# stateless-consensus/phant

Hardware: NVIDIA H100
Metric: mpt_proofs_verified_per_sec (higher is better)
Workload: dtype u64

## Files before the change

### phant_b200/csrc/abi.cu

```cuda
#include "../../include/phant_gpu.h"
#include "common.cuh"
#include "ctx.cuh"

#include <cub/device/device_scan.cuh>

#include <stdio.h>
#include <stdlib.h>
#include <string.h>
#include <new>

using namespace phant;

#define CU(expr)                                                              \
    do {                                                                      \
        cudaError_t e_ = (expr);                                              \
        if (e_ != cudaSuccess) return ctx->fail(e_, #expr, __FILE__, __LINE__); \
    } while (0)

int phant_gpu_ctx::fail(cudaError_t e, const char* what, const char* file, int line)
{
    snprintf(last_error, sizeof last_error, "%s: %s (%s:%d)", cudaGetErrorName(e), what, file, line);
    cudaGetLastError();
    return e == cudaErrorMemoryAllocation ? PHANT_GPU_E_OOM : PHANT_GPU_E_CUDA;
}
// ... 190 lines not shown
    stats.launches++;
    stats.keccak_msgs += n;
    stats.keccak_bytes += total_bytes;
    return PHANT_GPU_OK;
}

int phant_gpu_ctx::hash_slots(const uint8_t* d_msgs, const uint64_t* d_off, const uint64_t* d_len, uint64_t n, uint8_t* d_out)
{
    phant_gpu_ctx* ctx = this;
    if (n == 0) return PHANT_GPU_OK;
    KeccakVariant variant = KECCAK_STAGED;
    if (flags & PHANT_GPU_FLAG_KECCAK_DIRECT) variant = KECCAK_DIRECT;
    if (flags & PHANT_GPU_FLAG_KECCAK_WARP) variant = KECCAK_WARP;
    if (variant == KECCAK_STAGED && ((uintptr_t)d_msgs & 15)) variant = KECCAK_DIRECT;
    time_begin(0);
    CU(launch_keccak(stream, device, variant, d_msgs, d_off, nullptr, n, d_out, nullptr, d_len));
    time_end();
    stats.launches++;
    stats.keccak_msgs += n;
    return PHANT_GPU_OK;
}

bool phant_gpu_ctx::fused_ok(const uint8_t* d_nodes, uint64_t n_proofs, uint64_t n_nodes) const
{
    const uint32_t other = PHANT_GPU_FLAG_UNFUSED_WALK | PHANT_GPU_FLAG_KECCAK_DIRECT | PHANT_GPU_FLAG_KECCAK_WARP;
    return !(flags & other) && !((uintptr_t)d_nodes & 15) && !walk_peer && n_proofs <= 0xffffffffull && n_nodes <= 0xffffffffull;
}

int phant_gpu_ctx::verify_fused(const uint8_t* d_nodes, const uint64_t* d_node_off, uint64_t n_nodes, uint64_t total_bytes,
                                const uint64_t* d_proof_first, uint64_t np, const uint8_t* d_keys, const uint8_t* d_roots, uint64_t n_roots,
                                uint64_t* d_bitmap, uint8_t* d_status, uint64_t* d_voff, uint32_t* d_vlen)
{
    phant_gpu_ctx* ctx = this;
    if (np == 0) return wait_walk_fence();
    NvtxRange nvtx("phant:hash+walk");
    if (int rc = d_perms.reserve(ctx, 64)) return rc;
    if (!perms_init) { CU(cudaMemsetAsync(d_perms.ptr, 0, 64, stream)); perms_init = true; }
    const uint32_t* order = nullptr;
    if (!(flags & PHANT_GPU_FLAG_NO_BINNING) && np >= 4096) {
        if (int rc = d_idx.reserve(ctx, keccak_regroup_scratch_bytes(device, np))) return rc;
        if (int rc = d_order.reserve(ctx, 4 * np)) return rc;
        CU(launch_keccak_classify(stream, device, d_proof_first, np, (uint32_t*)d_idx.ptr, (uint32_t*)((unsigned long long*)d_perms.ptr + 1),
                                  nullptr, true));
        CU(launch_keccak_regroup(stream, device, d_proof_first, np, (const uint32_t*)d_idx.ptr, (uint32_t*)d_order.ptr, true));
        stats.launches += 2;
        order = (const uint32_t*)d_order.ptr;
    }
    if (!d_status) {
        if (int rc = ctx->d_status.reserve(ctx, np)) return rc;
        d_status = (uint8_t*)ctx->d_status.ptr;
    }
    time_begin(0);
    CU(launch_verify_fused(stream, device, d_nodes, d_node_off, d_proof_first, order, np, d_keys, d_roots, n_roots, d_status, d_voff, d_vlen,
                           (unsigned long long*)d_perms.ptr));
    time_end();
    stats.launches++;
    stats.keccak_msgs += n_nodes;
    stats.keccak_bytes += total_bytes;
    perms_pending = true;
    if (int rc = wait_walk_fence()) return rc;
    if (d_bitmap) {
        time_begin(1);
        CU(launch_verdict(stream, device, d_status, np, d_bitmap));
        time_end();
        stats.launches++;
    }
    return PHANT_GPU_OK;
}

static int check_offsets_host(const uint64_t* off, uint64_t n, uint64_t* total)
{
    for (uint64_t i = 0; i < n; ++i)
        if (off[i + 1] < off[i]) return PHANT_GPU_E_INVALID;
    *total = off[n];
    return PHANT_GPU_OK;
}

extern "C" int phant_gpu_keccak256_batch(phant_gpu_ctx* ctx, const uint8_t* msgs, const uint64_t* off, uint64_t n, uint8_t* out)
{
    if (!ctx || (n && (!off || !out))) return PHANT_GPU_E_INVALID;
    if (n == 0) return PHANT_GPU_OK;
    CU(cudaSetDevice(ctx->device));
    if (ctx->flags & PHANT_GPU_FLAG_DEVICE_PTRS) {
        uint64_t last = 0;
        CU(cudaMemcpyAsync(&last, off + n, 8, cudaMemcpyDeviceToHost, ctx->stream));
        CU(cudaStreamSynchronize(ctx->stream));
        if (last && !msgs) return PHANT_GPU_E_INVALID;
        return ctx->hash_csr(msgs, off, n, last, out);
    }
    uint64_t total = 0;
    if (int rc = check_offsets_host(off, n, &total)) return rc;
    if (total && !msgs) return PHANT_GPU_E_INVALID;
    if (int rc = ctx->d_msgs.reserve(ctx, total + 64)) return rc;
    if (int rc = ctx->d_off.reserve(ctx, 8 * (n + 1))) return rc;
    if (int rc = ctx->d_out.reserve(ctx, 32 * n)) return rc;
    if (total) CU(cudaMemcpyAsync(ctx->d_msgs.ptr, msgs, total, cudaMemcpyHostToDevice, ctx->stream));
    CU(cudaMemcpyAsync(ctx->d_off.ptr, off, 8 * (n + 1), cudaMemcpyHostToDevice, ctx->stream));
    ctx->stats.h2d_bytes += total + 8 * (n + 1);
    if (int rc = ctx->hash_csr((const uint8_t*)ctx->d_msgs.ptr, (const uint64_t*)ctx->d_off.ptr, n, total, (uint8_t*)ctx->d_out.ptr)) return rc;
    CU(cudaMemcpyAsync(out, ctx->d_out.ptr, 32 * n, cudaMemcpyDeviceToHost, ctx->stream));
    ctx->stats.d2h_bytes += 32 * n;
    CU(cudaStreamSynchronize(ctx->stream));
    return PHANT_GPU_OK;
}

extern "C" int phant_gpu_keccak256_batch_async(phant_gpu_ctx* ctx, const uint8_t* msgs, const uint64_t* off, uint64_t n, uint64_t total_bytes,
                                               uint8_t* out)
// ... 501 lines not shown
```

### phant_b200/csrc/common.cuh

```cuda
#pragma once
#include <cuda_runtime.h>
#include <stdint.h>

namespace phant {

enum KeccakVariant { KECCAK_STAGED = 0, KECCAK_DIRECT = 1, KECCAK_WARP = 2 };

int keccak_num_sms(int device);
cudaError_t launch_keccak(cudaStream_t s, int device, KeccakVariant variant, const uint8_t* msgs, const uint64_t* off,
                          const uint32_t* order, uint64_t n, uint8_t* out, uint32_t* summary ,
                          const uint64_t* len = nullptr );
uint64_t keccak_regroup_scratch_bytes(int device, uint64_t n);
cudaError_t launch_keccak_classify(cudaStream_t s, int device, const uint64_t* off, uint64_t n, uint32_t* hist, uint32_t* ticket,
                                   unsigned long long* perms, bool proofs = false);
cudaError_t launch_keccak_regroup(cudaStream_t s, int device, const uint64_t* off, uint64_t n, const uint32_t* start, uint32_t* order,
                                  bool proofs = false);
cudaError_t launch_verify_fused(cudaStream_t s, int device, const uint8_t* nodes, const uint64_t* node_off, const uint64_t* proof_first,
                                const uint32_t* order, uint64_t n, const uint8_t* keys32, const uint8_t* roots32, uint64_t n_roots,
                                uint8_t* status, uint64_t* val_off , uint32_t* val_len , unsigned long long* perms);

constexpr int PEER_MAX_WORLD = 16;
struct PeerOut {
    uint32_t* dst[PEER_MAX_WORLD];
    unsigned long long* ready[PEER_MAX_WORLD];
    const unsigned long long* done;
    unsigned long long wait_done;
    unsigned long long step;
    uint32_t* ticket;
    uint32_t* err;
    uint32_t world;
};

cudaError_t launch_walk(cudaStream_t s, int device, uint64_t n_proofs, const uint8_t* nodes, const uint64_t* node_off,
                        const uint64_t* node_index , const uint64_t* proof_first, const uint8_t* keys32, const uint8_t* roots32, uint64_t n_roots,
                        const uint8_t* digests, const uint32_t* summary , uint64_t* bitmap, uint8_t* status,
                        uint64_t* val_off, uint32_t* val_len, const PeerOut* peer = nullptr );

cudaError_t launch_verdict(cudaStream_t s, int device, const uint8_t* status, uint64_t n, uint64_t* bitmap);

cudaError_t launch_peer_collect(cudaStream_t s, const unsigned long long* ready, uint32_t world, unsigned long long step, const void* src, void* dst,
                                uint64_t bytes, const PeerOut& sig);

cudaError_t launch_bag_build(cudaStream_t s, int device, const uint8_t* digests, uint64_t n_nodes, uint32_t* table, uint32_t capacity);
cudaError_t launch_walk_bag(cudaStream_t s, int device, uint64_t n_keys, const uint8_t* nodes, const uint64_t* node_off, const uint8_t* keys32,
                            const uint8_t* roots32, uint64_t n_roots, const uint8_t* digests, const uint32_t* summary, const uint32_t* table,
                            uint32_t capacity, uint64_t* bitmap, uint8_t* status, uint64_t* val_off, uint32_t* val_len);

struct StateOut {
    uint8_t* account_status;
    uint64_t* nonce;
    uint8_t* balance32;
    uint8_t* storage_root32;
    uint8_t* code_hash32;
    uint32_t* code_index;
    uint8_t* slot_status;
    uint8_t* slot_vals32;
};
cudaError_t launch_read_accounts(cudaStream_t s, int device, uint64_t n_accounts, const uint8_t* nodes, const uint64_t* node_off,
                                 const uint8_t* digests, const uint32_t* summary, const uint32_t* table, uint32_t capacity,
                                 const uint8_t* keys32, const uint8_t* roots32, uint64_t n_roots, const uint8_t* code_digests,
                                 const uint32_t* code_table , uint32_t code_capacity, uint8_t* rec_roots32,
                                 uint8_t* rec_status, const StateOut& out);
cudaError_t launch_read_slots(cudaStream_t s, int device, uint64_t n_slots, const uint8_t* nodes, const uint64_t* node_off,
                              const uint8_t* digests, const uint32_t* summary, const uint32_t* table, uint32_t capacity,
                              const uint8_t* keys32, const uint32_t* slot_account, uint64_t n_accounts, const uint8_t* rec_roots32,
                              const uint8_t* rec_status, const StateOut& out);

cudaError_t launch_synth_c2(cudaStream_t s, int device, uint64_t seed, uint64_t first_index, uint64_t n, uint32_t depth,
                            int corrupt, uint8_t* nodes, uint64_t* node_off, uint64_t* proof_first, uint8_t* keys32,
                            uint8_t* roots32);
cudaError_t launch_synth_c3_sizes(cudaStream_t s, int device, uint64_t seed, uint64_t first_index, uint64_t n,
                                  uint64_t* n_nodes_per, uint64_t* n_bytes_per);
// ... 7 lines not shown
```

### phant_b200/csrc/keccak_f1600.cuh

```cuda
#pragma once
#include <stdint.h>

namespace phant {

__constant__ uint64_t KECCAK_RC[24] = {
    0x0000000000000001ull, 0x0000000000008082ull, 0x800000000000808aull, 0x8000000080008000ull,
    0x000000000000808bull, 0x0000000080000001ull, 0x8000000080008081ull, 0x8000000000008009ull,
    0x000000000000008aull, 0x0000000000000088ull, 0x0000000080008009ull, 0x000000008000000aull,
    0x000000008000808bull, 0x800000000000008bull, 0x8000000000008089ull, 0x8000000000008003ull,
    0x8000000000008002ull, 0x8000000000000080ull, 0x000000000000800aull, 0x800000008000000aull,
    0x8000000080008081ull, 0x8000000000008080ull, 0x0000000080000001ull, 0x8000000080008008ull};

constexpr int KECCAK_RATE = 136;
constexpr int KECCAK_RATE_WORDS = 17;

template <int N>
__device__ __forceinline__ uint64_t rol64(uint64_t x)
{
    if constexpr (N == 0) return x;
    const uint32_t lo = (uint32_t)x, hi = (uint32_t)(x >> 32);
    uint32_t rlo, rhi;
    if constexpr (N == 32) {
        rlo = hi; rhi = lo;
    } else if constexpr (N < 32) {
// ... 65 lines not shown
__device__ __forceinline__ MsgView msg_view(const void* p)
{
    const uintptr_t a = (uintptr_t)p;
    return MsgView{(const uint64_t*)(a & ~(uintptr_t)7), (uint32_t)(a & 7) * 8};
}
__device__ __forceinline__ uint64_t funnel64(uint64_t lo, uint64_t hi, uint32_t sh)
{
    return sh ? (lo >> sh) | (hi << (64 - sh)) : lo;
}

template <int UNROLL>
__device__ __forceinline__ void absorb_full(uint64_t (&st)[25], const MsgView& v, uint32_t base)
{
    uint64_t w[KECCAK_RATE_WORDS + 1];
#pragma unroll
    for (int k = 0; k < KECCAK_RATE_WORDS; ++k) w[k] = v.w[base + k];
    w[KECCAK_RATE_WORDS] = v.sh ? v.w[base + KECCAK_RATE_WORDS] : 0;
#pragma unroll
    for (int k = 0; k < KECCAK_RATE_WORDS; ++k) st[k] ^= funnel64(w[k], w[k + 1], v.sh);
    keccak_f1600<UNROLL>(st);
}

template <int UNROLL>
__device__ __forceinline__ void absorb_final(uint64_t (&st)[25], const MsgView& v, uint32_t base, uint32_t rem)
{
    const uint32_t mis = v.sh >> 3;
#pragma unroll
    for (int k = 0; k < KECCAK_RATE_WORDS; ++k) {
        const int valid = (int)rem - 8 * k;
        uint64_t word = 0;
        if (valid > 0) {
            const uint64_t lo = v.w[base + k];
            const uint64_t hi = (mis + (valid > 8 ? 8 : valid) > 8) ? v.w[base + k + 1] : 0;
            word = funnel64(lo, hi, v.sh);
            if (valid < 8) word &= (1ull << (8 * valid)) - 1;
        }
        if (valid >= 0 && valid < 8) word ^= 1ull << (8 * valid);
        st[k] ^= word;
    }
    st[KECCAK_RATE_WORDS - 1] ^= 0x8000000000000000ull;
    keccak_f1600<UNROLL, true>(st);
}

#ifndef PHANT_HOST_SMEM
__device__ __forceinline__ uint32_t lds32(uint32_t saddr)
{
    uint32_t v;
    asm volatile("ld.shared.u32 %0, [%1];" : "=r"(v) : "r"(saddr));
    return v;
}
#else
__device__ __forceinline__ uint32_t lds32(uint32_t saddr) { uint32_t v; memcpy(&v, PHANT_HOST_SMEM + saddr, 4); return v; }
#endif
template <int UNROLL, bool DIGEST_ONLY = false>
__device__ __forceinline__ void absorb_full_smem(uint64_t (&st)[25], uint32_t sa)
{
    const uint32_t a4 = sa & ~3u, sh = (sa & 3u) * 8;
    uint32_t w[2 * KECCAK_RATE_WORDS + 1];
#pragma unroll
    for (int j = 0; j < 2 * KECCAK_RATE_WORDS; ++j) w[j] = lds32(a4 + 4 * j);
    w[2 * KECCAK_RATE_WORDS] = sh ? lds32(a4 + 4 * 2 * KECCAK_RATE_WORDS) : 0;
#pragma unroll
    for (int k = 0; k < KECCAK_RATE_WORDS; ++k) {
        const uint32_t lo = __funnelshift_r(w[2 * k], w[2 * k + 1], sh);
        const uint32_t hi = __funnelshift_r(w[2 * k + 1], w[2 * k + 2], sh);
        st[k] ^= ((uint64_t)hi << 32) | lo;
    }
    keccak_f1600<UNROLL, DIGEST_ONLY>(st);
}
#ifndef PHANT_HOST_SMEM
__device__ __forceinline__ void sts32_(uint32_t saddr, uint32_t v) { asm volatile("st.shared.u32 [%0], %1;" ::"r"(saddr), "r"(v) : "memory"); }
#else
__device__ __forceinline__ void sts32_(uint32_t saddr, uint32_t v) { memcpy(PHANT_HOST_SMEM + saddr, &v, 4); }
#endif
template <int UNROLL>
__device__ __forceinline__ void absorb_final_smem_masked(uint64_t (&st)[25], uint32_t sa, uint32_t rem)
{
    const uint32_t a4 = sa & ~3u, sh = (sa & 3u) * 8;
    const uint32_t nfw = rem >> 2, tail = rem & 3u;
    const uint32_t bmask = (1u << (8 * tail)) - 1u, pad = 1u << (8 * tail);
    uint32_t prev = rem ? lds32(a4) : 0;
#pragma unroll
    for (int j = 0; j < 2 * KECCAK_RATE_WORDS; ++j) {
        uint32_t word = 0;
        if ((uint32_t)j < nfw || ((uint32_t)j == nfw && tail)) {
            const uint32_t next = lds32(a4 + 4 * (j + 1));
            word = __funnelshift_r(prev, next, sh);
            prev = next;
        }
        if ((uint32_t)j == nfw) word = (word & bmask) ^ pad;
        if (j == 2 * KECCAK_RATE_WORDS - 1) word ^= 0x80000000u;
        st[j >> 1] ^= (j & 1) ? ((uint64_t)word << 32) : (uint64_t)word;
    }
    keccak_f1600<UNROLL, true>(st);
}
template <int UNROLL>
__device__ __forceinline__ void absorb_final_smem(uint64_t (&st)[25], uint32_t sa, uint32_t rem, uint32_t room)
{
    if (room < KECCAK_RATE + 4) { absorb_final_smem_masked<UNROLL>(st, sa, rem); return; }
    const uint32_t a4 = sa & ~3u, s = sa & 3u;
    const uint32_t p0 = rem + s, p1 = KECCAK_RATE - 1 + s;
    const uint32_t q0 = p0 >> 2, b0 = p0 & 3u, q1 = p1 >> 2, b1 = p1 & 3u;
    uint32_t w0 = lds32(a4 + 4 * q0);
    w0 = (w0 & ((1u << (8 * b0)) - 1u)) | (1u << (8 * b0));
    if (q0 == q1) w0 |= 0x80u << (8 * b1);
    sts32_(a4 + 4 * q0, w0);
    for (uint32_t q = q0 + 1; q < q1; ++q) sts32_(a4 + 4 * q, 0u);
    if (q1 > q0) sts32_(a4 + 4 * q1, 0x80u << (8 * b1));
    absorb_full_smem<UNROLL, true>(st, sa);
}

template <int UNROLL = 2>
__device__ __forceinline__ void keccak256_thread(const uint8_t* p, uint64_t len, uint64_t (&digest)[4])
{
    uint64_t st[25];
#pragma unroll
    for (int i = 0; i < 25; ++i) st[i] = 0;
    const MsgView v = msg_view(p);
    uint32_t base = 0;
    while (len >= KECCAK_RATE) {
        absorb_full<UNROLL>(st, v, base);
        base += KECCAK_RATE_WORDS;
        len -= KECCAK_RATE;
    }
    absorb_final<UNROLL>(st, v, base, (uint32_t)len);
#pragma unroll
    for (int i = 0; i < 4; ++i) digest[i] = st[i];
}

}
```

### phant_b200/csrc/verify_fused.cu

```cuda
#include "common.cuh"
#include "stage.cuh"
#include "verify_fused.cuh"

namespace phant {

template <int UNROLL, int BLOCKS, int WARPS>
__global__ void __launch_bounds__(WARPS * 32)
verify_fused_kernel(const uint8_t* __restrict__ nodes, const uint64_t* __restrict__ node_off, const uint64_t* __restrict__ proof_first,
                    const uint32_t* __restrict__ order, uint64_t n, const uint8_t* __restrict__ keys32, const uint8_t* __restrict__ roots32,
                    uint64_t n_roots, uint8_t* __restrict__ status, uint64_t* __restrict__ val_off, uint32_t* __restrict__ val_len,
                    unsigned long long* __restrict__ perms)
{
    extern __shared__ __align__(128) uint8_t smem[];
    const uint32_t warp = threadIdx.x >> 5, lane = threadIdx.x & 31;
    const uint32_t bar = smem_u32(smem) + 8 * warp;
    constexpr int SLOT = stage_slot(BLOCKS), WINDOW = stage_window(BLOCKS);
    uint8_t* slot = smem + 128 + (warp * 32 + lane) * SLOT;
    const uint32_t slot_s = smem_u32(slot);
    if (lane == 0) mbar_init(bar, 32);
    fence_proxy_async();
    __syncthreads();
    uint32_t parity = 0;
    unsigned long long my_perms = 0;

    const uint64_t n_tiles = (n + 31) / 32;
    for (uint64_t tile = (uint64_t)blockIdx.x * WARPS + warp; tile < n_tiles; tile += (uint64_t)gridDim.x * WARPS) {
        const uint64_t idx = tile * 32 + lane;
        const bool active = idx < n;
        uint64_t p = 0;
        FusedLane L;
        L.done = true;
        if (active) {
            p = order ? order[idx] : idx;
            fused_begin(L, node_off, proof_first[p], proof_first[p + 1], keys32 + 32 * p, roots32 + (n_roots == 1 ? 0 : 32 * p));
        }
        while (!__all_sync(0xffffffffu, L.done)) {
            uint64_t a0 = 0;
            const uint32_t cs = L.done ? 0 : fused_window<WINDOW>(L, a0);
            if (cs) {
                fence_proxy_async();
                mbar_arrive_expect_tx(bar, cs);
                bulk_g2s(slot_s, nodes + a0, cs, bar);
            } else {
                mbar_arrive(bar);
            }
            mbar_wait(bar, parity);
            parity ^= 1;
            if (!L.done) fused_step<UNROLL, SLOT>(L, nodes, node_off, slot_s, slot, cs);
        }
        if (active) {
            status[p] = (uint8_t)L.status;
            if (val_off) val_off[p] = L.voff;
            if (val_len) val_len[p] = L.vlen;
            my_perms += L.perms;
        }
    }
    for (int o = 16; o; o >>= 1) my_perms += __shfl_down_sync(0xffffffffu, my_perms, o);
    if (lane == 0 && my_perms) atomicAdd(perms, my_perms);
}

cudaError_t launch_verify_fused(cudaStream_t s, int device, const uint8_t* nodes, const uint64_t* node_off, const uint64_t* proof_first,
                                const uint32_t* order, uint64_t n, const uint8_t* keys32, const uint8_t* roots32, uint64_t n_roots,
                                uint8_t* status, uint64_t* val_off, uint32_t* val_len, unsigned long long* perms)
{
    if (n == 0) return cudaSuccess;
    constexpr int BLOCKS = 4, WARPS = 12;
    constexpr int SMEM = stage_smem(BLOCKS, WARPS);
    static int ctas_cache[64] = {0};
    int& ctas_per_sm = ctas_cache[(device >= 0 && device < 64) ? device : 0];
    if (!ctas_per_sm) {
        cudaError_t e = cudaFuncSetAttribute(verify_fused_kernel<2, BLOCKS, WARPS>, cudaFuncAttributeMaxDynamicSharedMemorySize, SMEM);
        if (e != cudaSuccess) return e;
        cudaFuncSetAttribute(verify_fused_kernel<2, BLOCKS, WARPS>, cudaFuncAttributePreferredSharedMemoryCarveout, 100);
        e = cudaOccupancyMaxActiveBlocksPerMultiprocessor(&ctas_per_sm, verify_fused_kernel<2, BLOCKS, WARPS>, WARPS * 32, SMEM);
        if (e != cudaSuccess || ctas_per_sm < 1) { ctas_per_sm = 0; return e != cudaSuccess ? e : cudaErrorLaunchOutOfResources; }
    }
    const uint64_t tiles = (n + 31) / 32;
    uint64_t blocks = (tiles + WARPS - 1) / WARPS;
    const uint64_t cap = (uint64_t)keccak_num_sms(device) * ctas_per_sm;
    if (blocks > cap) blocks = cap;
    verify_fused_kernel<2, BLOCKS, WARPS><<<(unsigned)blocks, WARPS * 32, SMEM, s>>>(nodes, node_off, proof_first, order, n, keys32, roots32,
                                                                                    n_roots, status, val_off, val_len, perms);
    return cudaGetLastError();
}


}
```

### phant_b200/csrc/verify_fused.cuh

```cuda
#pragma once
#include <stdint.h>

#include "keccak_f1600.cuh"
#include "node_summary.cuh"
#include "walk_one.cuh"

namespace phant {
namespace {

struct FusedLane {
    uint64_t st[25];
    uint32_t expect[8];
    uint32_t kw[8];
    uint32_t pos;
    uint64_t i, last;
    uint64_t cur, end;
    uint64_t voff;
    uint32_t vlen;
    uint64_t perms;
    int status;
    bool done;
    bool fresh;
};

__device__ __forceinline__ uint64_t node_perms(uint64_t len) { return len / KECCAK_RATE + 1; }

__device__ __forceinline__ void fused_finish(FusedLane& L, const uint64_t* __restrict__ node_off, int status)
{
    L.status = status;
    L.done = true;
    for (uint64_t j = L.i + 1; j < L.last; ++j) L.perms += node_perms(node_off[j + 1] - node_off[j]);
}

__device__ __forceinline__ void fused_enter(FusedLane& L, const uint64_t* __restrict__ node_off)
{
    L.cur = node_off[L.i];
    L.end = node_off[L.i + 1];
#pragma unroll
    for (int k = 0; k < 25; ++k) L.st[k] = 0;
    L.fresh = true;
    L.perms += node_perms(L.end - L.cur);
    if (L.end - L.cur > 0xffffffffull) fused_finish(L, node_off, ST_REJECT);
}

__device__ __forceinline__ void fused_begin(FusedLane& L, const uint64_t* __restrict__ node_off, uint64_t first, uint64_t last,
                                            const uint8_t* __restrict__ key, const uint8_t* __restrict__ root)
{
    L.voff = 0;
    L.vlen = 0;
    L.perms = 0;
    L.pos = 0;
    L.done = false;
    L.status = ST_REJECT;
    load32_aligned(root, L.expect);
    load32_aligned(key, L.kw);
    L.i = first;
    L.last = last;
    if (first == last) {
        L.status = eq32_const(EMPTY_ROOT, L.expect) ? ST_ABSENT : ST_REJECT;
        L.done = true;
        return;
    }
    fused_enter(L, node_off);
}

template <int WINDOW>
__device__ __forceinline__ uint32_t fused_window(const FusedLane& L, uint64_t& a0)
{
    a0 = L.cur & ~(uint64_t)15;
    if (L.end == L.cur) return 0;
    const uint64_t span = ((L.end - a0) + 15) & ~(uint64_t)15;
    return span < (uint64_t)WINDOW ? (uint32_t)span : (uint32_t)WINDOW;
}

template <int UNROLL, int SLOT>
__device__ __forceinline__ void fused_step(FusedLane& L, const uint8_t* __restrict__ nodes, const uint64_t* __restrict__ node_off,
                                           uint32_t slot_s, const uint8_t* slot, uint32_t cs)
{
    const uint64_t need = L.end - L.cur;
    const uint32_t skew = (uint32_t)(L.cur & 15);
    const uint64_t in_slot = (uint64_t)cs - skew;
    const uint64_t avail = need < in_slot ? need : in_slot;
    const uint32_t nfull = (uint32_t)(avail / KECCAK_RATE);
    uint32_t sa = slot_s + skew;
    for (uint32_t b = 0; b < nfull; ++b) {
        absorb_full_smem<UNROLL>(L.st, sa);
        sa += KECCAK_RATE;
    }
    if (avail != need) {
        L.cur += (uint64_t)nfull * KECCAK_RATE;
        L.fresh = false;
        return;
    }
    absorb_final_smem<UNROLL>(L.st, sa, (uint32_t)(avail - (uint64_t)nfull * KECCAK_RATE), slot_s + SLOT - sa);
    uint32_t diff = 0;
#pragma unroll
    for (int k = 0; k < 4; ++k) diff |= ((uint32_t)L.st[k] ^ L.expect[2 * k]) | ((uint32_t)(L.st[k] >> 32) ^ L.expect[2 * k + 1]);
    if (diff) { fused_finish(L, node_off, ST_REJECT); return; }
    const bool is_last = L.i + 1 == L.last;
    const uint64_t beg = L.fresh ? L.cur : node_off[L.i];
    const uint32_t len = (uint32_t)(L.end - beg);
    const uint32_t sm = L.fresh ? summarize_node(slot + skew, len) : 0;
    int r;
    if ((sm & 3u) == 1u && L.pos < 64) {
        const uint32_t nibble = key_nibble(L.kw, L.pos);
        ++L.pos;
        const uint32_t mask = sm >> 8;
        if (!((mask >> nibble) & 1u)) { fused_finish(L, node_off, is_last ? ST_ABSENT : ST_REJECT); return; }
        const uint32_t before = __popc(mask & ((1u << nibble) - 1u));
        const uint32_t ra = slot_s + skew + ((sm >> 2) & 7u) + 33u * before + (nibble - before) + 1u;
        const uint32_t a4 = ra & ~3u, sh = (ra & 3u) * 8;
        uint32_t w[9];
#pragma unroll
        for (int k = 0; k < 9; ++k) w[k] = lds32(a4 + 4 * k);
#pragma unroll
        for (int k = 0; k < 8; ++k) L.expect[k] = __funnelshift_r(w[k], w[k + 1], sh);
        r = WALK_NEXT;
    } else {
        r = walk_node(nodes, nodes + beg, len, 0, is_last, L.kw, L.pos, L.expect, L.voff, L.vlen);
    }
    if (r != WALK_NEXT) { fused_finish(L, node_off, r); return; }
    if (is_last) { fused_finish(L, node_off, ST_REJECT); return; }
    ++L.i;
    fused_enter(L, node_off);
}

}
}
```

### phant_b200/csrc/stage.cuh

```cuda
#pragma once
#include <stdint.h>

#include "keccak_f1600.cuh"

namespace phant {

constexpr int stage_window(int blocks)
{
    int s = (blocks * KECCAK_RATE + 15 + 15) / 16;
    if (s % 2 == 0) ++s;
    return 16 * s;
}
constexpr int stage_slot(int blocks) { return stage_window(blocks) + 32; }
constexpr int stage_smem(int blocks, int warps) { return 128 + warps * 32 * stage_slot(blocks) + 16; }
static_assert(stage_smem(4, 12) <= 232448, "default shape must fit the 227 KB a CTA may opt into");

__device__ __forceinline__ uint32_t smem_u32(const void* p) { return (uint32_t)__cvta_generic_to_shared(p); }
__device__ __forceinline__ void mbar_init(uint32_t bar, uint32_t count)
{
    asm volatile("mbarrier.init.shared::cta.b64 [%0], %1;" ::"r"(bar), "r"(count));
}
__device__ __forceinline__ void mbar_arrive(uint32_t bar)
{
    asm volatile("mbarrier.arrive.shared::cta.b64 _, [%0];" ::"r"(bar) : "memory");
}
__device__ __forceinline__ void mbar_arrive_expect_tx(uint32_t bar, uint32_t bytes)
{
    asm volatile("mbarrier.arrive.expect_tx.shared::cta.b64 _, [%0], %1;" ::"r"(bar), "r"(bytes) : "memory");
}
__device__ __forceinline__ void mbar_wait(uint32_t bar, uint32_t parity)
{
    asm volatile(
        "{\n"
        ".reg .pred P1;\n"
        "LAB_WAIT:\n"
        "mbarrier.try_wait.parity.shared::cta.b64 P1, [%0], %1;\n"
        "@P1 bra DONE;\n"
        "bra LAB_WAIT;\n"
        "DONE:\n"
        "}" ::"r"(bar), "r"(parity) : "memory");
}
__device__ __forceinline__ void bulk_g2s(uint32_t dst, const void* src, uint32_t bytes, uint32_t bar)
{
    asm volatile("cp.async.bulk.shared::cluster.global.mbarrier::complete_tx::bytes [%0], [%1], %2, [%3];"
                 ::"r"(dst), "l"(src), "r"(bytes), "r"(bar) : "memory");
}
__device__ __forceinline__ void fence_proxy_async() { asm volatile("fence.proxy.async.shared::cta;" ::: "memory"); }

}
```

Measured before the change: 121.3 million.

## Overlap next-window bulk copy with final Keccak permutation and add dynamic tile scheduling

Splits each fused step into an absorb phase, which XORs the block and extracts the child reference into shared memory, and a complete phase, which runs the last permutation and the walk. The next TMA bulk copy (next window, next node, or the first window of the next tile) is issued between the two phases, so the copy overlaps the final keccak. It also replaces the static grid-stride tile loop with atomic-counter work stealing that resets itself at kernel end, and adds a fast path for 4-byte-aligned shared-memory XOR. The cost is more control flow, extra register pressure, and warp-wide shuffles and atomics per tile.

```diff
diff --git a/phant_b200/csrc/abi.cu b/phant_b200/csrc/abi.cu
--- a/phant_b200/csrc/abi.cu
+++ b/phant_b200/csrc/abi.cu
@@ -266,7 +266,7 @@
     }
     time_begin(0);
     CU(launch_verify_fused(stream, device, d_nodes, d_node_off, d_proof_first, order, np, d_keys, d_roots, n_roots, d_status, d_voff, d_vlen,
-                           (unsigned long long*)d_perms.ptr));
+                           (unsigned long long*)d_perms.ptr, (uint32_t*)((unsigned long long*)d_perms.ptr + 2)));
     time_end();
     stats.launches++;
     stats.keccak_msgs += n_nodes;
diff --git a/phant_b200/csrc/common.cuh b/phant_b200/csrc/common.cuh
--- a/phant_b200/csrc/common.cuh
+++ b/phant_b200/csrc/common.cuh
@@ -17,7 +17,8 @@
                                   bool proofs = false);
 cudaError_t launch_verify_fused(cudaStream_t s, int device, const uint8_t* nodes, const uint64_t* node_off, const uint64_t* proof_first,
                                 const uint32_t* order, uint64_t n, const uint8_t* keys32, const uint8_t* roots32, uint64_t n_roots,
-                                uint8_t* status, uint64_t* val_off , uint32_t* val_len , unsigned long long* perms);
+                                uint8_t* status, uint64_t* val_off , uint32_t* val_len , unsigned long long* perms,
+                                uint32_t* tiles);
 
 constexpr int PEER_MAX_WORLD = 16;
 struct PeerOut {
diff --git a/phant_b200/csrc/keccak_f1600.cuh b/phant_b200/csrc/keccak_f1600.cuh
--- a/phant_b200/csrc/keccak_f1600.cuh
+++ b/phant_b200/csrc/keccak_f1600.cuh
@@ -141,8 +141,7 @@
 #else
 __device__ __forceinline__ uint32_t lds32(uint32_t saddr) { uint32_t v; memcpy(&v, PHANT_HOST_SMEM + saddr, 4); return v; }
 #endif
-template <int UNROLL, bool DIGEST_ONLY = false>
-__device__ __forceinline__ void absorb_full_smem(uint64_t (&st)[25], uint32_t sa)
+__device__ __forceinline__ void xor_block_smem(uint64_t (&st)[25], uint32_t sa)
 {
     const uint32_t a4 = sa & ~3u, sh = (sa & 3u) * 8;
     uint32_t w[2 * KECCAK_RATE_WORDS + 1];
@@ -155,6 +154,21 @@
         const uint32_t hi = __funnelshift_r(w[2 * k + 1], w[2 * k + 2], sh);
         st[k] ^= ((uint64_t)hi << 32) | lo;
     }
+}
+__device__ __forceinline__ void xor_block_smem_aligned(uint64_t (&st)[25], uint32_t sa)
+{
+#pragma unroll
+    for (int k = 0; k < KECCAK_RATE_WORDS; ++k) st[k] ^= ((uint64_t)lds32(sa + 8 * k + 4) << 32) | lds32(sa + 8 * k);
+}
+__device__ __forceinline__ void xor_block_smem(uint64_t (&st)[25], uint32_t sa, bool aligned)
+{
+    if (aligned) xor_block_smem_aligned(st, sa);
+    else xor_block_smem(st, sa);
+}
+template <int UNROLL, bool DIGEST_ONLY = false>
+__device__ __forceinline__ void absorb_full_smem(uint64_t (&st)[25], uint32_t sa)
+{
+    xor_block_smem(st, sa);
     keccak_f1600<UNROLL, DIGEST_ONLY>(st);
 }
 #ifndef PHANT_HOST_SMEM
@@ -162,8 +176,7 @@
 #else
 __device__ __forceinline__ void sts32_(uint32_t saddr, uint32_t v) { memcpy(PHANT_HOST_SMEM + saddr, &v, 4); }
 #endif
-template <int UNROLL>
-__device__ __forceinline__ void absorb_final_smem_masked(uint64_t (&st)[25], uint32_t sa, uint32_t rem)
+__device__ __forceinline__ void xor_final_smem_masked(uint64_t (&st)[25], uint32_t sa, uint32_t rem)
 {
     const uint32_t a4 = sa & ~3u, sh = (sa & 3u) * 8;
     const uint32_t nfw = rem >> 2, tail = rem & 3u;
@@ -181,12 +194,15 @@
         if (j == 2 * KECCAK_RATE_WORDS - 1) word ^= 0x80000000u;
         st[j >> 1] ^= (j & 1) ? ((uint64_t)word << 32) : (uint64_t)word;
     }
+}
+template <int UNROLL>
+__device__ __forceinline__ void absorb_final_smem_masked(uint64_t (&st)[25], uint32_t sa, uint32_t rem)
+{
+    xor_final_smem_masked(st, sa, rem);
     keccak_f1600<UNROLL, true>(st);
 }
-template <int UNROLL>
-__device__ __forceinline__ void absorb_final_smem(uint64_t (&st)[25], uint32_t sa, uint32_t rem, uint32_t room)
-{
-    if (room < KECCAK_RATE + 4) { absorb_final_smem_masked<UNROLL>(st, sa, rem); return; }
+__device__ __forceinline__ void pad_final_smem(uint32_t sa, uint32_t rem)
+{
     const uint32_t a4 = sa & ~3u, s = sa & 3u;
     const uint32_t p0 = rem + s, p1 = KECCAK_RATE - 1 + s;
     const uint32_t q0 = p0 >> 2, b0 = p0 & 3u, q1 = p1 >> 2, b1 = p1 & 3u;
@@ -196,7 +212,19 @@
     sts32_(a4 + 4 * q0, w0);
     for (uint32_t q = q0 + 1; q < q1; ++q) sts32_(a4 + 4 * q, 0u);
     if (q1 > q0) sts32_(a4 + 4 * q1, 0x80u << (8 * b1));
+}
+template <int UNROLL>
+__device__ __forceinline__ void absorb_final_smem(uint64_t (&st)[25], uint32_t sa, uint32_t rem, uint32_t room)
+{
+    if (room < KECCAK_RATE + 4) { absorb_final_smem_masked<UNROLL>(st, sa, rem); return; }
+    pad_final_smem(sa, rem);
     absorb_full_smem<UNROLL, true>(st, sa);
+}
+__device__ __forceinline__ void xor_final_smem(uint64_t (&st)[25], uint32_t sa, uint32_t rem, uint32_t room, bool aligned)
+{
+    if (room < KECCAK_RATE + 4) { xor_final_smem_masked(st, sa, rem); return; }
+    pad_final_smem(sa, rem);
+    xor_block_smem(st, sa, aligned);
 }
 
 template <int UNROLL = 2>
diff --git a/phant_b200/csrc/verify_fused.cu b/phant_b200/csrc/verify_fused.cu
--- a/phant_b200/csrc/verify_fused.cu
+++ b/phant_b200/csrc/verify_fused.cu
@@ -4,12 +4,19 @@
 
 namespace phant {
 
+#ifdef PHANT_FUSED_STALLS
+constexpr int FUSED_STALLS_WARPS = 8192;
+__device__ unsigned long long phant_fused_stalls[FUSED_STALLS_WARPS][8];
+#endif
+
+constexpr uint32_t NO_WINDOW = 0xffffffffu;
+
 template <int UNROLL, int BLOCKS, int WARPS>
 __global__ void __launch_bounds__(WARPS * 32)
 verify_fused_kernel(const uint8_t* __restrict__ nodes, const uint64_t* __restrict__ node_off, const uint64_t* __restrict__ proof_first,
                     const uint32_t* __restrict__ order, uint64_t n, const uint8_t* __restrict__ keys32, const uint8_t* __restrict__ roots32,
                     uint64_t n_roots, uint8_t* __restrict__ status, uint64_t* __restrict__ val_off, uint32_t* __restrict__ val_len,
-                    unsigned long long* __restrict__ perms)
+                    unsigned long long* __restrict__ perms, uint32_t* __restrict__ tiles)
 {
     extern __shared__ __align__(128) uint8_t smem[];
     const uint32_t warp = threadIdx.x >> 5, lane = threadIdx.x & 31;
@@ -22,46 +29,122 @@
     __syncthreads();
     uint32_t parity = 0;
     unsigned long long my_perms = 0;
+#ifdef PHANT_FUSED_STALLS
+    unsigned long long wait_first = 0, wait_other = 0, trips_first = 0, trips_other = 0;
+    const long long t_loop = clock64();
+#endif
 
     const uint64_t n_tiles = (n + 31) / 32;
-    for (uint64_t tile = (uint64_t)blockIdx.x * WARPS + warp; tile < n_tiles; tile += (uint64_t)gridDim.x * WARPS) {
+    const uint64_t first_dyn = (uint64_t)gridDim.x * WARPS;
+    const auto take_tile = [&]() -> uint64_t {
+        uint32_t t = 0;
+        if (lane == 0) t = atomicAdd(&tiles[0], 1u);
+        return first_dyn + __shfl_sync(0xffffffffu, t, 0);
+    };
+    uint64_t tile = (uint64_t)blockIdx.x * WARPS + warp;
+    uint64_t next = tile < n_tiles ? take_tile() : n_tiles;
+    const auto issue = [&](uint32_t cs, uint64_t a0) {
+        if (cs) {
+            fence_proxy_async();
+            mbar_arrive_expect_tx(bar, cs);
+            bulk_g2s(slot_s, nodes + a0, cs, bar);
+        } else {
+            mbar_arrive(bar);
+        }
+    };
+
+    FusedLane L;
+    uint64_t p = 0;
+    const auto begin = [&]() {
         const uint64_t idx = tile * 32 + lane;
-        const bool active = idx < n;
-        uint64_t p = 0;
-        FusedLane L;
         L.done = true;
-        if (active) {
+        if (tile < n_tiles && idx < n) {
             p = order ? order[idx] : idx;
             fused_begin(L, node_off, proof_first[p], proof_first[p + 1], keys32 + 32 * p, roots32 + (n_roots == 1 ? 0 : 32 * p));
         }
-        while (!__all_sync(0xffffffffu, L.done)) {
-            uint64_t a0 = 0;
-            const uint32_t cs = L.done ? 0 : fused_window<WINDOW>(L, a0);
-            if (cs) {
-                fence_proxy_async();
-                mbar_arrive_expect_tx(bar, cs);
-                bulk_g2s(slot_s, nodes + a0, cs, bar);
-            } else {
-                mbar_arrive(bar);
-            }
+    };
+    begin();
+    uint32_t cs_now = NO_WINDOW, cs_ahead = NO_WINDOW;
+    {
+        uint64_t a0 = 0;
+        const uint32_t cs = L.done ? 0 : fused_window<WINDOW>(L, a0);
+        issue(cs, a0);
+        if (!L.done) cs_now = cs;
+    }
+    while (tile < n_tiles) {
+#ifdef PHANT_FUSED_STALLS
+        int first_trip = 1;
+#endif
+        for (;;) {
+#ifdef PHANT_FUSED_STALLS
+            const long long t0 = clock64();
+#endif
             mbar_wait(bar, parity);
             parity ^= 1;
-            if (!L.done) fused_step<UNROLL, SLOT>(L, nodes, node_off, slot_s, slot, cs);
+#ifdef PHANT_FUSED_STALLS
+            const unsigned long long dt = (unsigned long long)(clock64() - t0);
+            if (first_trip) { wait_first += dt; ++trips_first; } else { wait_other += dt; ++trips_other; }
+            first_trip = 0;
+#endif
+            const bool work = !L.done && cs_now != NO_WINDOW;
+            const bool aligned = __all_sync(0xffffffffu, !work || (L.cur & 3) == 0);
+            const uint32_t kind = work ? fused_absorb<UNROLL, SLOT>(L, slot_s, slot, cs_now, aligned) : FT_CONT;
+            uint64_t a0 = 0;
+            uint32_t cs = 0, cs_next = NO_WINDOW;
+            if (!L.done && !work) {
+                cs = fused_window<WINDOW>(L, a0);
+                cs_next = cs;
+            } else if (work && (kind == FT_CONT || L.i + 1 < L.last)) {
+                cs = fused_next_window<WINDOW>(L, node_off, kind, a0);
+                cs_next = cs;
+            } else if (cs_ahead == NO_WINDOW) {
+                const uint64_t idx = next * 32 + lane;
+                if (next < n_tiles && idx < n) cs = fused_first_window<WINDOW>(node_off, proof_first, order ? order[idx] : idx, a0);
+                cs_ahead = cs;
+            }
+            issue(cs, a0);
+            if (work) fused_complete<UNROLL, SLOT>(L, nodes, node_off, slot_s, kind);
+            cs_now = cs_next;
+            if (__all_sync(0xffffffffu, L.done)) break;
         }
-        if (active) {
+        if (tile * 32 + lane < n) {
             status[p] = (uint8_t)L.status;
             if (val_off) val_off[p] = L.voff;
             if (val_len) val_len[p] = L.vlen;
             my_perms += L.perms;
         }
+        tile = next;
+        if (tile < n_tiles) next = take_tile();
+        begin();
+        cs_now = cs_ahead;
+        cs_ahead = NO_WINDOW;
     }
+    mbar_wait(bar, parity);
+#ifdef PHANT_FUSED_STALLS
+    const uint64_t gw = (uint64_t)blockIdx.x * WARPS + warp;
+    if (lane == 0 && gw < FUSED_STALLS_WARPS) {
+        unsigned long long* o = phant_fused_stalls[gw];
+        o[0] = wait_first;
+        o[1] = wait_other;
+        o[2] = trips_first;
+        o[3] = trips_other;
+        o[4] = (unsigned long long)(clock64() - t_loop);
+    }
+#endif
     for (int o = 16; o; o >>= 1) my_perms += __shfl_down_sync(0xffffffffu, my_perms, o);
     if (lane == 0 && my_perms) atomicAdd(perms, my_perms);
+    if (lane == 0) {
+        __threadfence();
+        if (atomicAdd(&tiles[1], 1u) == first_dyn - 1) {
+            tiles[0] = 0;
+            tiles[1] = 0;
+        }
+    }
 }
 
 cudaError_t launch_verify_fused(cudaStream_t s, int device, const uint8_t* nodes, const uint64_t* node_off, const uint64_t* proof_first,
                                 const uint32_t* order, uint64_t n, const uint8_t* keys32, const uint8_t* roots32, uint64_t n_roots,
-                                uint8_t* status, uint64_t* val_off, uint32_t* val_len, unsigned long long* perms)
+                                uint8_t* status, uint64_t* val_off, uint32_t* val_len, unsigned long long* perms, uint32_t* tiles)
 {
     if (n == 0) return cudaSuccess;
     constexpr int BLOCKS = 4, WARPS = 12;
@@ -75,14 +158,25 @@
         e = cudaOccupancyMaxActiveBlocksPerMultiprocessor(&ctas_per_sm, verify_fused_kernel<2, BLOCKS, WARPS>, WARPS * 32, SMEM);
         if (e != cudaSuccess || ctas_per_sm < 1) { ctas_per_sm = 0; return e != cudaSuccess ? e : cudaErrorLaunchOutOfResources; }
     }
-    const uint64_t tiles = (n + 31) / 32;
-    uint64_t blocks = (tiles + WARPS - 1) / WARPS;
+    const uint64_t n_tiles = (n + 31) / 32;
+    uint64_t blocks = (n_tiles + WARPS - 1) / WARPS;
     const uint64_t cap = (uint64_t)keccak_num_sms(device) * ctas_per_sm;
     if (blocks > cap) blocks = cap;
     verify_fused_kernel<2, BLOCKS, WARPS><<<(unsigned)blocks, WARPS * 32, SMEM, s>>>(nodes, node_off, proof_first, order, n, keys32, roots32,
-                                                                                    n_roots, status, val_off, val_len, perms);
+                                                                                    n_roots, status, val_off, val_len, perms, tiles);
     return cudaGetLastError();
 }
 
+#ifdef PHANT_FUSED_STALLS
+extern "C" int phant_gpu_debug_fused_stalls(unsigned long long* out, int max_warps)
+{
+    const int w = max_warps < FUSED_STALLS_WARPS ? max_warps : FUSED_STALLS_WARPS;
+    if (cudaMemcpyFromSymbol(out, phant_fused_stalls, sizeof(unsigned long long) * 8 * w) != cudaSuccess) return -1;
+    static unsigned long long zero[FUSED_STALLS_WARPS][8];
+    if (cudaMemcpyToSymbol(phant_fused_stalls, zero, sizeof zero) != cudaSuccess) return -1;
+    return w;
+}
+#endif
+
 
 }
diff --git a/phant_b200/csrc/verify_fused.cuh b/phant_b200/csrc/verify_fused.cuh
--- a/phant_b200/csrc/verify_fused.cuh
+++ b/phant_b200/csrc/verify_fused.cuh
@@ -65,59 +65,105 @@
 }
 
 template <int WINDOW>
-__device__ __forceinline__ uint32_t fused_window(const FusedLane& L, uint64_t& a0)
+__device__ __forceinline__ uint32_t window_at(uint64_t cur, uint64_t end, uint64_t& a0)
 {
-    a0 = L.cur & ~(uint64_t)15;
-    if (L.end == L.cur) return 0;
-    const uint64_t span = ((L.end - a0) + 15) & ~(uint64_t)15;
+    a0 = cur & ~(uint64_t)15;
+    if (end == cur) return 0;
+    const uint64_t span = ((end - a0) + 15) & ~(uint64_t)15;
     return span < (uint64_t)WINDOW ? (uint32_t)span : (uint32_t)WINDOW;
 }
 
+template <int WINDOW>
+__device__ __forceinline__ uint32_t fused_window(const FusedLane& L, uint64_t& a0)
+{
+    return window_at<WINDOW>(L.cur, L.end, a0);
+}
+
+enum : uint32_t {
+    FT_CONT = 0,
+    FT_WALK = 1,
+    FT_REF = 2,
+    FT_NOREF = 3,
+};
+
 template <int UNROLL, int SLOT>
-__device__ __forceinline__ void fused_step(FusedLane& L, const uint8_t* __restrict__ nodes, const uint64_t* __restrict__ node_off,
-                                           uint32_t slot_s, const uint8_t* slot, uint32_t cs)
+__device__ __forceinline__ uint32_t fused_absorb(FusedLane& L, uint32_t slot_s, const uint8_t* slot, uint32_t cs, bool aligned)
 {
     const uint64_t need = L.end - L.cur;
     const uint32_t skew = (uint32_t)(L.cur & 15);
     const uint64_t in_slot = (uint64_t)cs - skew;
     const uint64_t avail = need < in_slot ? need : in_slot;
     const uint32_t nfull = (uint32_t)(avail / KECCAK_RATE);
+    const bool ends = avail == need;
+    const uint32_t nperm = ends ? nfull : nfull - 1;
     uint32_t sa = slot_s + skew;
-    for (uint32_t b = 0; b < nfull; ++b) {
-        absorb_full_smem<UNROLL>(L.st, sa);
+    for (uint32_t b = 0; b < nperm; ++b) {
+        xor_block_smem(L.st, sa, aligned);
+        keccak_f1600<UNROLL>(L.st);
         sa += KECCAK_RATE;
     }
-    if (avail != need) {
+    if (!ends) {
+        xor_block_smem(L.st, sa, aligned);
         L.cur += (uint64_t)nfull * KECCAK_RATE;
         L.fresh = false;
-        return;
+        return FT_CONT;
     }
-    absorb_final_smem<UNROLL>(L.st, sa, (uint32_t)(avail - (uint64_t)nfull * KECCAK_RATE), slot_s + SLOT - sa);
+    xor_final_smem(L.st, sa, (uint32_t)(avail - (uint64_t)nfull * KECCAK_RATE), slot_s + SLOT - sa, aligned);
+    const uint32_t sm = L.fresh ? summarize_node(slot + skew, (uint32_t)need) : 0;
+    if ((sm & 3u) != 1u || L.pos >= 64) return FT_WALK;
+    const uint32_t nibble = key_nibble(L.kw, L.pos);
+    ++L.pos;
+    const uint32_t mask = sm >> 8;
+    if (!((mask >> nibble) & 1u)) return FT_NOREF;
+    const uint32_t before = __popc(mask & ((1u << nibble) - 1u));
+    const uint32_t ra = slot_s + skew + ((sm >> 2) & 7u) + 33u * before + (nibble - before) + 1u;
+    const uint32_t a4 = ra & ~3u, sh = (ra & 3u) * 8;
+    uint32_t w[9];
+#pragma unroll
+    for (int k = 0; k < 9; ++k) w[k] = lds32(a4 + 4 * k);
+#pragma unroll
+    for (int k = 0; k < 8; ++k) sts32_(slot_s + SLOT - 32 + 4 * k, __funnelshift_r(w[k], w[k + 1], sh));
+    return FT_REF;
+}
+
+template <int WINDOW>
+__device__ __forceinline__ uint32_t fused_next_window(const FusedLane& L, const uint64_t* __restrict__ node_off, uint32_t kind, uint64_t& a0)
+{
+    if (kind == FT_CONT) return fused_window<WINDOW>(L, a0);
+    return window_at<WINDOW>(node_off[L.i + 1], node_off[L.i + 2], a0);
+}
+
+template <int WINDOW>
+__device__ __forceinline__ uint32_t fused_first_window(const uint64_t* __restrict__ node_off, const uint64_t* __restrict__ proof_first,
+                                                       uint64_t p, uint64_t& a0)
+{
+    const uint64_t first = proof_first[p];
+    a0 = 0;
+    if (first == proof_first[p + 1]) return 0;
+    return window_at<WINDOW>(node_off[first], node_off[first + 1], a0);
+}
+
+template <int UNROLL, int SLOT>
+__device__ __forceinline__ void fused_complete(FusedLane& L, const uint8_t* __restrict__ nodes, const uint64_t* __restrict__ node_off,
+                                               uint32_t slot_s, uint32_t kind)
+{
+    if (kind == FT_CONT) { keccak_f1600<UNROLL>(L.st); return; }
+    keccak_f1600<UNROLL, true>(L.st);
     uint32_t diff = 0;
 #pragma unroll
     for (int k = 0; k < 4; ++k) diff |= ((uint32_t)L.st[k] ^ L.expect[2 * k]) | ((uint32_t)(L.st[k] >> 32) ^ L.expect[2 * k + 1]);
     if (diff) { fused_finish(L, node_off, ST_REJECT); return; }
     const bool is_last = L.i + 1 == L.last;
-    const uint64_t beg = L.fresh ? L.cur : node_off[L.i];
-    const uint32_t len = (uint32_t)(L.end - beg);
-    const uint32_t sm = L.fresh ? summarize_node(slot + skew, len) : 0;
     int r;
-    if ((sm & 3u) == 1u && L.pos < 64) {
-        const uint32_t nibble = key_nibble(L.kw, L.pos);
-        ++L.pos;
-        const uint32_t mask = sm >> 8;
-        if (!((mask >> nibble) & 1u)) { fused_finish(L, node_off, is_last ? ST_ABSENT : ST_REJECT); return; }
-        const uint32_t before = __popc(mask & ((1u << nibble) - 1u));
-        const uint32_t ra = slot_s + skew + ((sm >> 2) & 7u) + 33u * before + (nibble - before) + 1u;
-        const uint32_t a4 = ra & ~3u, sh = (ra & 3u) * 8;
-        uint32_t w[9];
+    if (kind == FT_REF) {
 #pragma unroll
-        for (int k = 0; k < 9; ++k) w[k] = lds32(a4 + 4 * k);
-#pragma unroll
-        for (int k = 0; k < 8; ++k) L.expect[k] = __funnelshift_r(w[k], w[k + 1], sh);
+        for (int k = 0; k < 8; ++k) L.expect[k] = lds32(slot_s + SLOT - 32 + 4 * k);
         r = WALK_NEXT;
+    } else if (kind == FT_NOREF) {
+        r = is_last ? ST_ABSENT : ST_REJECT;
     } else {
-        r = walk_node(nodes, nodes + beg, len, 0, is_last, L.kw, L.pos, L.expect, L.voff, L.vlen);
+        const uint64_t beg = L.fresh ? L.cur : node_off[L.i];
+        r = walk_node(nodes, nodes + beg, (uint32_t)(L.end - beg), 0, is_last, L.kw, L.pos, L.expect, L.voff, L.vlen);
     }
     if (r != WALK_NEXT) { fused_finish(L, node_off, r); return; }
     if (is_last) { fused_finish(L, node_off, ST_REJECT); return; }
@@ -125,5 +171,13 @@
     fused_enter(L, node_off);
 }
 
+template <int UNROLL, int SLOT>
+__device__ __forceinline__ void fused_step(FusedLane& L, const uint8_t* __restrict__ nodes, const uint64_t* __restrict__ node_off,
+                                           uint32_t slot_s, const uint8_t* slot, uint32_t cs)
+{
+    const uint32_t kind = fused_absorb<UNROLL, SLOT>(L, slot_s, slot, cs, (L.cur & 3) == 0);
+    fused_complete<UNROLL, SLOT>(L, nodes, node_off, slot_s, kind);
+}
+
 }
 }
```

Result: no change. 121.8 million (median of 6 runs) (+0.4%).

## Replace per-warp TMA bulk copies with per-lane cp.async and add aligned absorb path

Applied to the files above, without the earlier changes.

Each lane now stages its node window with 16-byte cp.async copies and waits with cp.async.wait_all. This replaces the per-warp mbarrier, expect-tx and bulk_g2s handshake, along with its init, fence and block-wide sync. Keccak absorption gains a warp-uniform fast path for 8-byte-aligned input that skips the funnel-shift realignment. On the first block of a node it loads the rate words straight into the state, so the state zeroing moves out of fused_enter. The cost is more copy instructions per lane and reliance on the first-block flag to reset the state correctly.

```diff
diff --git a/phant_b200/csrc/keccak_f1600.cuh b/phant_b200/csrc/keccak_f1600.cuh
--- a/phant_b200/csrc/keccak_f1600.cuh
+++ b/phant_b200/csrc/keccak_f1600.cuh
@@ -141,19 +141,40 @@
 #else
 __device__ __forceinline__ uint32_t lds32(uint32_t saddr) { uint32_t v; memcpy(&v, PHANT_HOST_SMEM + saddr, 4); return v; }
 #endif
-template <int UNROLL, bool DIGEST_ONLY = false>
-__device__ __forceinline__ void absorb_full_smem(uint64_t (&st)[25], uint32_t sa)
+#if defined(__CUDACC__) && !defined(PHANT_HOST_SMEM)
+__device__ __forceinline__ bool warp_all_active(bool p) { return __all_sync(__activemask(), p); }
+#else
+__device__ __forceinline__ bool warp_all_active(bool p) { return p; }
+#endif
+template <int UNROLL, bool DIGEST_ONLY = false, bool WORD_PATH = false>
+__device__ __forceinline__ void absorb_full_smem(uint64_t (&st)[25], uint32_t sa, bool first = false)
 {
     const uint32_t a4 = sa & ~3u, sh = (sa & 3u) * 8;
-    uint32_t w[2 * KECCAK_RATE_WORDS + 1];
-#pragma unroll
-    for (int j = 0; j < 2 * KECCAK_RATE_WORDS; ++j) w[j] = lds32(a4 + 4 * j);
-    w[2 * KECCAK_RATE_WORDS] = sh ? lds32(a4 + 4 * 2 * KECCAK_RATE_WORDS) : 0;
-#pragma unroll
-    for (int k = 0; k < KECCAK_RATE_WORDS; ++k) {
-        const uint32_t lo = __funnelshift_r(w[2 * k], w[2 * k + 1], sh);
-        const uint32_t hi = __funnelshift_r(w[2 * k + 1], w[2 * k + 2], sh);
-        st[k] ^= ((uint64_t)hi << 32) | lo;
+    if (WORD_PATH && warp_all_active(sh == 0 && first)) {
+#pragma unroll
+        for (int k = 0; k < KECCAK_RATE_WORDS; ++k) st[k] = ((uint64_t)lds32(a4 + 8 * k + 4) << 32) | lds32(a4 + 8 * k);
+#pragma unroll
+        for (int k = KECCAK_RATE_WORDS; k < 25; ++k) st[k] = 0;
+    } else {
+        if (WORD_PATH && first) {
+#pragma unroll
+            for (int k = 0; k < 25; ++k) st[k] = 0;
+        }
+        if (WORD_PATH && warp_all_active(sh == 0)) {
+#pragma unroll
+            for (int k = 0; k < KECCAK_RATE_WORDS; ++k) st[k] ^= ((uint64_t)lds32(a4 + 8 * k + 4) << 32) | lds32(a4 + 8 * k);
+        } else {
+            uint32_t w[2 * KECCAK_RATE_WORDS + 1];
+#pragma unroll
+            for (int j = 0; j < 2 * KECCAK_RATE_WORDS; ++j) w[j] = lds32(a4 + 4 * j);
+            w[2 * KECCAK_RATE_WORDS] = sh ? lds32(a4 + 4 * 2 * KECCAK_RATE_WORDS) : 0;
+#pragma unroll
+            for (int k = 0; k < KECCAK_RATE_WORDS; ++k) {
+                const uint32_t lo = __funnelshift_r(w[2 * k], w[2 * k + 1], sh);
+                const uint32_t hi = __funnelshift_r(w[2 * k + 1], w[2 * k + 2], sh);
+                st[k] ^= ((uint64_t)hi << 32) | lo;
+            }
+        }
     }
     keccak_f1600<UNROLL, DIGEST_ONLY>(st);
 }
@@ -183,10 +204,17 @@
     }
     keccak_f1600<UNROLL, true>(st);
 }
-template <int UNROLL>
-__device__ __forceinline__ void absorb_final_smem(uint64_t (&st)[25], uint32_t sa, uint32_t rem, uint32_t room)
-{
-    if (room < KECCAK_RATE + 4) { absorb_final_smem_masked<UNROLL>(st, sa, rem); return; }
+template <int UNROLL, bool WORD_PATH = false>
+__device__ __forceinline__ void absorb_final_smem(uint64_t (&st)[25], uint32_t sa, uint32_t rem, uint32_t room, bool first = false)
+{
+    if (room < KECCAK_RATE + 4) {
+        if (WORD_PATH && first) {
+#pragma unroll
+            for (int k = 0; k < 25; ++k) st[k] = 0;
+        }
+        absorb_final_smem_masked<UNROLL>(st, sa, rem);
+        return;
+    }
     const uint32_t a4 = sa & ~3u, s = sa & 3u;
     const uint32_t p0 = rem + s, p1 = KECCAK_RATE - 1 + s;
     const uint32_t q0 = p0 >> 2, b0 = p0 & 3u, q1 = p1 >> 2, b1 = p1 & 3u;
@@ -196,7 +224,7 @@
     sts32_(a4 + 4 * q0, w0);
     for (uint32_t q = q0 + 1; q < q1; ++q) sts32_(a4 + 4 * q, 0u);
     if (q1 > q0) sts32_(a4 + 4 * q1, 0x80u << (8 * b1));
-    absorb_full_smem<UNROLL, true>(st, sa);
+    absorb_full_smem<UNROLL, true, WORD_PATH>(st, sa, first);
 }
 
 template <int UNROLL = 2>
diff --git a/phant_b200/csrc/stage.cuh b/phant_b200/csrc/stage.cuh
--- a/phant_b200/csrc/stage.cuh
+++ b/phant_b200/csrc/stage.cuh
@@ -47,4 +47,31 @@
 }
 __device__ __forceinline__ void fence_proxy_async() { asm volatile("fence.proxy.async.shared::cta;" ::: "memory"); }
 
+__device__ __forceinline__ void cp_async16(uint32_t dst, const uint8_t* src)
+{
+    asm volatile("cp.async.cg.shared.global [%0], [%1], 16;" ::"r"(dst), "l"(src) : "memory");
 }
+__device__ __forceinline__ void cp_async16_below(uint32_t dst, const uint8_t* src, uint32_t off, uint32_t bytes)
+{
+    asm volatile("{\n"
+                 ".reg .pred p;\n"
+                 "setp.lt.u32 p, %2, %3;\n"
+                 "@p cp.async.cg.shared.global [%0], [%1], 16;\n"
+                 "}" ::"r"(dst), "l"(src), "r"(off), "r"(bytes) : "memory");
+}
+template <int WINDOW>
+__device__ __forceinline__ void lane_g2s(uint32_t dst, const uint8_t* src, uint32_t bytes)
+{
+    constexpr int N = WINDOW / 16;
+    if (warp_all_active(bytes >= 16u * (N - 1))) {
+#pragma unroll
+        for (int k = 0; k < N - 1; ++k) cp_async16(dst + 16 * k, src + 16 * k);
+    } else {
+#pragma unroll
+        for (int k = 0; k < N - 1; ++k) cp_async16_below(dst + 16 * k, src + 16 * k, 16u * k, bytes);
+    }
+    cp_async16_below(dst + 16 * (N - 1), src + 16 * (N - 1), 16u * (N - 1), bytes);
+}
+__device__ __forceinline__ void lane_g2s_wait() { asm volatile("cp.async.wait_all;" ::: "memory"); }
+
+}
diff --git a/phant_b200/csrc/verify_fused.cu b/phant_b200/csrc/verify_fused.cu
--- a/phant_b200/csrc/verify_fused.cu
+++ b/phant_b200/csrc/verify_fused.cu
@@ -13,14 +13,9 @@
 {
     extern __shared__ __align__(128) uint8_t smem[];
     const uint32_t warp = threadIdx.x >> 5, lane = threadIdx.x & 31;
-    const uint32_t bar = smem_u32(smem) + 8 * warp;
     constexpr int SLOT = stage_slot(BLOCKS), WINDOW = stage_window(BLOCKS);
     uint8_t* slot = smem + 128 + (warp * 32 + lane) * SLOT;
     const uint32_t slot_s = smem_u32(slot);
-    if (lane == 0) mbar_init(bar, 32);
-    fence_proxy_async();
-    __syncthreads();
-    uint32_t parity = 0;
     unsigned long long my_perms = 0;
 
     const uint64_t n_tiles = (n + 31) / 32;
@@ -37,15 +32,8 @@
         while (!__all_sync(0xffffffffu, L.done)) {
             uint64_t a0 = 0;
             const uint32_t cs = L.done ? 0 : fused_window<WINDOW>(L, a0);
-            if (cs) {
-                fence_proxy_async();
-                mbar_arrive_expect_tx(bar, cs);
-                bulk_g2s(slot_s, nodes + a0, cs, bar);
-            } else {
-                mbar_arrive(bar);
-            }
-            mbar_wait(bar, parity);
-            parity ^= 1;
+            lane_g2s<WINDOW>(slot_s, nodes + a0, cs);
+            lane_g2s_wait();
             if (!L.done) fused_step<UNROLL, SLOT>(L, nodes, node_off, slot_s, slot, cs);
         }
         if (active) {
diff --git a/phant_b200/csrc/verify_fused.cuh b/phant_b200/csrc/verify_fused.cuh
--- a/phant_b200/csrc/verify_fused.cuh
+++ b/phant_b200/csrc/verify_fused.cuh
@@ -36,8 +36,6 @@
 {
     L.cur = node_off[L.i];
     L.end = node_off[L.i + 1];
-#pragma unroll
-    for (int k = 0; k < 25; ++k) L.st[k] = 0;
     L.fresh = true;
     L.perms += node_perms(L.end - L.cur);
     if (L.end - L.cur > 0xffffffffull) fused_finish(L, node_off, ST_REJECT);
@@ -84,7 +82,7 @@
     const uint32_t nfull = (uint32_t)(avail / KECCAK_RATE);
     uint32_t sa = slot_s + skew;
     for (uint32_t b = 0; b < nfull; ++b) {
-        absorb_full_smem<UNROLL>(L.st, sa);
+        absorb_full_smem<UNROLL, false, true>(L.st, sa, L.fresh && b == 0);
         sa += KECCAK_RATE;
     }
     if (avail != need) {
@@ -92,7 +90,7 @@
         L.fresh = false;
         return;
     }
-    absorb_final_smem<UNROLL>(L.st, sa, (uint32_t)(avail - (uint64_t)nfull * KECCAK_RATE), slot_s + SLOT - sa);
+    absorb_final_smem<UNROLL, true>(L.st, sa, (uint32_t)(avail - (uint64_t)nfull * KECCAK_RATE), slot_s + SLOT - sa, L.fresh && nfull == 0);
     uint32_t diff = 0;
 #pragma unroll
     for (int k = 0; k < 4; ++k) diff |= ((uint32_t)L.st[k] ^ L.expect[2 * k]) | ((uint32_t)(L.st[k] >> 32) ^ L.expect[2 * k + 1]);
```

Result: faster. 124.1 million before, 125.9 million after (median of 6 runs) (+1.5%).
